# pwrliang/RayJoin

Hardware: AMD Instinct MI355X
Metric: LSI+PIP query throughput, USCounty |><| BlockGroup (higher is better)
Workload: dtype int128+f64; 1 GPU; USCounty(base, 7112768 segs) |><| BlockGroup(query, 28793160 segs, 29665680 points), -query=lsi then -query=pip, -mode=lbvh (software LBVH); kernel_schedule=k_lsi and the PIP kernels share the chip (512 + 1536 blocks), schedule_settled_before_timing=True

## Files before the change

rayjoin_amd/csrc/rj_api.hip:

```cpp
#include <hip/hip_runtime.h>
#include <rccl/rccl.h>

#include <cmath>
#include <cstdarg>
#include <cstdio>
#include <cstring>
#include <functional>
#include <new>
#include <string>
#include <thread>
#include <vector>

#include "../../include/rayjoin_amd.h"
#include "rj_crossings.h"
#include "rj_dissolve.h"
#include "rj_eliminate.h"
#include "rj_faces.h"
#include "rj_node.h"
#include "rj_kernels.h"
#include "rj_overlay_dev.h"
#include "rj_overlay_ops.h"
#include "rj_pipeline.h"
#include "rj_polygons.h"
#include "rj_ringmap.h"
// ... 1815 lines not shown
    }
  const char* why = !h->pip_walk ? "\"pip_walk\" 0: the exact kernel alone" : (walk ? "" : "instrumented (\"stats\"), no points, or more than 2^32 of them: the exact kernel alone");
  if (walk && h->pip_walk == 1 && seen != ~0ull && (seen * 10 > n * 3 || seen > 16384)) {
    walk = false;
    why = "the last two-pass query of this size left too many points to the exact kernel (> 30 %, or > 16384): first pass dropped";
  }
  const bool own = aux && walk && h->exact_own_stream;
  const int li = own ? 1 + h->exact_buf : si;
  if (walk && (h->rest_cap[si] < n || h->rest_cap[li] < n)) {
    RJ_HIP(h, hipStreamSynchronize(h->stream));
    RJ_HIP(h, join_aux(h));
    for (int k = 0; k < (h->exact_own_stream ? 3 : 2); k++) {
      if (h->rest_cap[k] >= n) continue;
      (void) hipFree(h->rest[k]); (void) hipFree(h->todo[k]); (void) hipFree(h->todo_mask[k]);
      h->rest[k] = nullptr; h->rest_cap[k] = 0; h->todo[k] = nullptr; h->todo_mask[k] = nullptr;
      if (int r = dev_alloc(h, &h->rest[k], n)) return r;
      if (int r = dev_alloc(h, &h->todo[k], n * (uint64_t) pip_walk_list_slots())) return r;
      if (int r = dev_alloc(h, &h->todo_mask[k], n / 4 + 1)) return r;
      h->rest_cap[k] = n;
      RJ_HIP(h, hipMemsetAsync(h->todo[k], 0xFF, n * (uint64_t) pip_walk_list_slots() * 4, h->stream));
      RJ_HIP(h, hipMemsetAsync(h->todo_mask[k], 0, (n / 4 + 1) * 8, h->stream));
      RJ_HIP(h, hipMemsetAsync(h->rest[k], 0, n * 4, h->stream));
    }
    RJ_HIP(h, hipStreamSynchronize(h->stream));
  }
  h->last_passes = walk ? 3 : 1;
  h->last_walk_points = 1;
  h->last_prepared = 0;
  tic(h, RJ_T_PIP_KERNEL, st);
  if (n && walk) {
    const int wflip = h->flip_walk[si];
    PipArgs w = a;
    w.work_counter = (unsigned int*) (h->d_counter + (aux ? kSchedWalkAux : kSchedWalkMain) + wflip * kSchedBlockWords);
    w.next_work_counter = (unsigned int*) (h->d_counter + (aux ? kSchedWalkAux : kSchedWalkMain) + (1 - wflip) * kSchedBlockWords);
    w.rest = h->rest[li];
    w.rest_count = h->d_counter + kRestCountWord + 2 * si + wflip;
    w.next_rest_count = h->d_counter + kRestCountWord + 2 * si + (1 - wflip);
    if (own) {
      w.rest_count = h->d_counter + kExactRestWord[h->exact_rot];
      w.next_rest_count = h->d_counter + kExactRestWord[(h->exact_rot + 1) % 3];
      h->exact_rot = (h->exact_rot + 1) % 3;
      if (h->exact_recorded[h->exact_buf]) RJ_HIP(h, hipStreamWaitEvent(st, h->ev_exact_done[h->exact_buf], 0));
      if (h->exact_last >= 0 && h->exact_recorded[h->exact_last] &&
          (h->exact_out_closest == (const void*) closest_eid_dev || (face_id_dev && h->exact_out_face == (const void*) face_id_dev)))
        RJ_HIP(h, hipStreamWaitEvent(st, h->ev_exact_done[h->exact_last], 0));
    }
    w.todo = h->todo[li]; w.todo_mask = h->todo_mask[li];
    if (!w.group_lanes) w.group_lanes = pip_walk_group_lanes(n, w.bvh.top, h->cus);
    const bool two = h->walk_points >= 2 && w.group_lanes == 64 && !h->chunk_groups && pip_walk2_blocks_per_cu(w.bvh.top) >= 6 &&
                     n >= (uint64_t) 2 * 256 * 4 * h->cus * pip_walk2_blocks_per_cu(w.bvh.top);
    tic(h, RJ_T_PIP_WALK, st);
    const bool columns = w.bvh.strips.ytab != nullptr;
    h->last_columns = columns ? 1 : 0;
    if (columns) {
      w.group_lanes = 64;
      RJ_HIP(h, launch_pip_strip(st, w, walk_blocks, h->cus));
    } else if (two) {
      if (aux && h->lsi_shared && !h->pip_share_set)
        walk_blocks = h->cus * pip_walk2_blocks_beside(w.bvh.top, walk_share_of_this_pair / h->cus < 1 ? 1 : walk_share_of_this_pair / h->cus);
      const MapState& q = h->map[query_map_id];
      if (!pts_dev && !order && !h->stats_on && q.qpts) {
        w.qpts = q.qpts + pt_begin;
        h->last_prepared = 1;
        if (pt_begin % 64 == 0) { w.qext = q.qext + pt_begin / 64; h->last_prepared = 2; }
      }
      RJ_HIP(h, launch_pip_walk2(st, w, walk_blocks, h->cus, h->stats_on));
      h->last_walk_points = 2;
    } else {
      RJ_HIP(h, launch_pip_walk(st, w, h->stats_on, walk_blocks));
    }
    if (aux && h->lsi_shared) h->last_pip_share = walk_blocks;
    h->plan.pip.first = columns ? last_strip_launch() : last_launch();
    toc(h, RJ_T_PIP_WALK, st);
    h->flip_walk[si] = 1 - wflip;
    const uint64_t left = seen != ~0ull ? seen : 8192;
    PipRestArgs r;
    r.order = h->rest[li];
    r.n_dev = w.rest_count;
    r.rest_count = h->d_rest + si;
    r.work_counter = a.work_counter;
    r.next_work_counter = a.next_work_counter;
    r.group_lanes = left < 8192 ? 1 : (left * 100 < n ? 4 : (left * 10 < n ? 8 : 16));
    r.chunk_groups = 1;
    int rest_blocks = h->cus * 4;
    if (seen != ~0ull) {
      const uint64_t want = seen / (r.group_lanes * 4 * 2) + 1;
      const uint64_t lo = (uint64_t) h->cus / 4, hi = (uint64_t) h->cus * 4;
      rest_blocks = (int) (want < lo ? lo : (want > hi ? hi : want));
    }
    r.blocks = (uint32_t) rest_blocks;
    h->walk_n[si] = n;
    if (own) {
      RJ_HIP(h, hipEventRecord(h->ev_walk_done, st));
      RJ_HIP(h, hipStreamWaitEvent(h->exact_stream, h->ev_walk_done, 0));
      RJ_HIP(h, launch_pip_exact(h->exact_stream, w, h->cus * 8, r));
      RJ_HIP(h, hipEventRecord(h->ev_exact_done[h->exact_buf], h->exact_stream));
      h->exact_recorded[h->exact_buf] = true;
      h->exact_last = h->exact_buf;
      h->exact_out_closest = closest_eid_dev; h->exact_out_face = face_id_dev;
      h->exact_buf ^= 1;
      h->exact_pending = true;
    } else {
      RJ_HIP(h, launch_pip_exact(st, w, h->cus * 8, r));
    }
    h->flip_pip[si] = 1 - pflip;
    h->plan.pip.exact_blocks = h->cus * 8; h->plan.pip.locate_blocks = rest_blocks;
    if (columns) why = "the base map has a column index (closed rings or short chains: index[].columns_why): the first pass reads the point's strip";
    else if (!two && h->walk_points >= 2) why = "one point per lane: a query set too small for full groups on every resident wave (or a debug knob set)";
  } else if (n) {
    if (aux && h->exact_pending && h->exact_last >= 0) RJ_HIP(h, hipStreamWaitEvent(st, h->ev_exact_done[h->exact_last], 0));
    RJ_HIP(h, launch_pip(st, a, h->stats_on, max_blocks));
    h->flip_pip[aux ? 1 : 0] = 1 - pflip;
    h->plan.pip.first = last_launch();
    h->plan.pip.exact_blocks = h->plan.pip.locate_blocks = 0;
  }
  {
    rj_handle_s::PlanRec::Pip& pp = h->plan.pip;
    pp.ran = n > 0; pp.epoch = h->plan.epoch; pp.n = n; pp.aux = aux; pp.caller = pts_dev != nullptr;
    pp.shared = aux && h->lsi_shared; pp.passes = h->last_passes; pp.rest_hint = seen; pp.why = why;
    pp.order = order ? (h->order_fresh ? 2 : 1) : 0;
    pp.prepared = h->last_prepared;
  }
  toc(h, RJ_T_PIP_KERNEL, own ? h->exact_stream : st);
  if (h->cur_caller >= 0 && n) {
    const rj_handle_s::CallerSet& e = h->caller[h->cur_caller];
    if (e.queries <= 2 || e.queries % 4 == 0) RJ_HIP(h, launch_group_extent_tail(st, pts, h->cur_order, n, h->d_est + h->cur_caller));
  }
  if (aux) h->aux_pending = true;
  return RJ_OK;
}

int rj_pip_query(rj_handle h, int base_map_id, int query_map_id, const int64_t* pts_dev,
                 uint64_t pt_begin, uint64_t n, uint32_t* closest_eid_dev, int32_t* face_id_dev) {
  RJ_CHECK_H(h);
  if (int r = rj_pip_query_async(h, base_map_id, query_map_id, pts_dev, pt_begin, n, closest_eid_dev, face_id_dev)) return r;
  if (h->stats_on) RJ_HIP(h, hipMemcpyAsync(h->h_pinned + 1, h->d_stats, 128, hipMemcpyDeviceToHost, h->stream));
  RJ_HIP(h, hipStreamSynchronize(h->stream));
  RJ_HIP(h, join_aux(h));
  if (h->stats_on) for (int i = 0; i < 16; i++) h->last_stats[i] = h->h_pinned[1 + i];
  return check_fault(h);
}


int rj_build_grid(rj_handle h, int map_id, int grid_size) {
  RJ_CHECK_H(h);
  if (map_id < 0 || map_id > 1 || !h->map[map_id].present) return fail(h, RJ_E_INVALID, "rj_build_grid: map %d not uploaded", map_id);
  if (grid_size < 1 || grid_size > 32768) return fail(h, RJ_E_INVALID, "rj_build_grid: grid_size must be in [1, 32768]");
  if (int r = set_device(h)) return r;
  RJ_HIP(h, join_aux(h));
  const MapState& m = h->map[map_id];
  GridState& gr = h->grid[map_id];
  free_grid(gr);
  const uint64_t ncells = (uint64_t) grid_size * grid_size;
  const double scale = (double) grid_size / (double) ((((int64_t) 1 << 46) - 1) + ((int64_t) 1 << 46)) * 0.999;
  tic(h, RJ_T_BUILD);
  uint32_t* counts = nullptr;
  uint64_t *keys = nullptr, *keys2 = nullptr;
  void* temp = nullptr;
  int rc = RJ_OK;
  hipError_t e = hipSuccess;
  do {
    if ((rc = dev_alloc(h, &counts, ncells + 1))) break;
    if ((rc = dev_alloc(h, &gr.begin, ncells + 1))) break;
    if ((e = hipMemsetAsync(counts, 0, (ncells + 1) * 4, h->stream)) != hipSuccess) break;
    if ((e = hipMemsetAsync(h->d_counter + 2, 0, 16, h->stream)) != hipSuccess) break;
    if ((e = launch_grid_count(h->stream, m.seg, m.ne, grid_size, scale, counts, h->d_counter + 2)) != hipSuccess) break;
    if ((e = hipMemcpyAsync(h->h_pinned + 26, h->d_counter + 2, 8, hipMemcpyDeviceToHost, h->stream)) != hipSuccess) break;
    if ((e = hipStreamSynchronize(h->stream)) != hipSuccess) break;
    gr.total = h->h_pinned[26];
    if (gr.total >= 0xFFFFFFFFull) {
      rc = fail(h, RJ_E_INVALID, "rj_build_grid: %llu (cell, edge) incidences do not fit 32-bit offsets: use a coarser grid",
                (unsigned long long) gr.total);
      break;
    }
    size_t scan_bytes = 0, sort_bytes = 0;
    if ((e = scan_cell_counts(h->stream, nullptr, scan_bytes, counts, gr.begin, ncells + 1)) != hipSuccess) break;
    if (gr.total && (e = sort_keys_u64(h->stream, nullptr, sort_bytes, (const uint64_t*) nullptr, (uint64_t*) nullptr, gr.total)) != hipSuccess) break;
    const size_t temp_bytes = scan_bytes > sort_bytes ? scan_bytes : sort_bytes;
    if ((e = hipMalloc(&temp, temp_bytes ? temp_bytes : 1)) != hipSuccess) break;
    size_t tb = temp_bytes;
    if ((e = scan_cell_counts(h->stream, temp, tb, counts, gr.begin, ncells + 1)) != hipSuccess) break;
    if ((rc = dev_alloc(h, &gr.eids, gr.total ? gr.total : 1))) break;
    if (gr.total) {
      if ((rc = dev_alloc(h, &keys, gr.total))) break;
      if ((rc = dev_alloc(h, &keys2, gr.total))) break;
      if ((e = launch_grid_emit(h->stream, m.seg, m.ne, grid_size, scale, keys, h->d_counter + 3)) != hipSuccess) break;
      tb = temp_bytes;
      if ((e = sort_keys_u64(h->stream, temp, tb, keys, keys2, gr.total)) != hipSuccess) break;
      if ((e = launch_grid_unpack(h->stream, keys2, gr.total, gr.eids)) != hipSuccess) break;
// ... 864 lines not shown
```

rayjoin_amd/csrc/rj_kernels.hip:

```cpp
#include "rj_kernels.h"

#include <cstring>
#include <rocprim/device/device_radix_sort.hpp>

namespace rj {

__device__ __forceinline__ uint32_t cell_code(const Seg& s) {
  const int cx0 = quant(s.x1 < s.x2 ? s.x1 : s.x2) >> kOccShift, cx1 = quant(s.x1 < s.x2 ? s.x2 : s.x1) >> kOccShift;
  const int cy0 = quant(s.y1 < s.y2 ? s.y1 : s.y2) >> kOccShift, cy1 = quant(s.y1 < s.y2 ? s.y2 : s.y1) >> kOccShift;
  const int dx = cx1 - cx0 > 1 ? 2 : cx1 - cx0, dy = cy1 - cy0 > 1 ? 2 : cy1 - cy0;
  return (uint32_t) cx0 | ((uint32_t) cy0 << 12) | ((uint32_t) dx << 24) | ((uint32_t) dy << 26);
}
__global__ __launch_bounds__(256) void k_build_segs(const int64_t* __restrict__ pts,
                                                    const uint32_t* __restrict__ edge_begin,
                                                    uint32_t nc, uint64_t ne, Seg* __restrict__ seg,
                                                    uint32_t* __restrict__ edge_chain, uint32_t* __restrict__ ccode) {
  for (uint64_t e = blockIdx.x * (uint64_t) blockDim.x + threadIdx.x; e < ne;
       e += (uint64_t) gridDim.x * blockDim.x) {
    uint32_t lo = 0, hi = nc;
    while (hi - lo > 1) {
      uint32_t mid = lo + ((hi - lo) >> 1);
      if (edge_begin[mid] <= e) lo = mid; else hi = mid;
    }
    uint64_t p = e + lo;
// ... 1124 lines not shown
}


__global__ __launch_bounds__(256) void k_xsect_keys(const XsectRec* __restrict__ rec, uint64_t n, int im,
                                                    uint64_t* __restrict__ keys, uint32_t* __restrict__ vals) {
  for (uint64_t i = blockIdx.x * (uint64_t) blockDim.x + threadIdx.x; i < n; i += (uint64_t) gridDim.x * blockDim.x) {
    const uint32_t mine = im ? rec[i].eid1 : rec[i].eid0, other = im ? rec[i].eid0 : rec[i].eid1;
    keys[i] = ((uint64_t) mine << 32) | other;
    vals[i] = (uint32_t) i;
  }
}

__global__ __launch_bounds__(256) void k_xsect_gather(const XsectRec* __restrict__ in, const uint32_t* __restrict__ order,
                                                      uint64_t n, XsectRec* __restrict__ out) {
  for (uint64_t i = blockIdx.x * (uint64_t) blockDim.x + threadIdx.x; i < n; i += (uint64_t) gridDim.x * blockDim.x)
    out[i] = in[order[i]];
}

__device__ __forceinline__ u128 xsect_dist2(const XsectRec& r, int64_t px, int64_t py) {
  const i128 dx = (i128) r.x_num - px, dy = (i128) r.y_num - py;
  return (u128) (dx * dx) + (u128) (dy * dy);
}

__global__ __launch_bounds__(256) void k_xsect_order_runs(XsectRec* __restrict__ rec, uint64_t n, int im,
                                                          const Seg* __restrict__ seg_im,
                                                          int64_t* __restrict__ midpts) {
  for (uint64_t i = blockIdx.x * (uint64_t) blockDim.x + threadIdx.x; i < n; i += (uint64_t) gridDim.x * blockDim.x) {
    const uint32_t e = im ? rec[i].eid1 : rec[i].eid0;
    if (i > 0 && (im ? rec[i - 1].eid1 : rec[i - 1].eid0) == e) continue;
    uint64_t end = i + 1;
    while (end < n && (im ? rec[end].eid1 : rec[end].eid0) == e) end++;
    const Seg s = seg_im[e];
    for (uint64_t a = i + 1; a < end; a++) {
      const XsectRec cur = rec[a];
      const u128 dc = xsect_dist2(cur, s.x1, s.y1);
      uint64_t b = a;
      while (b > i && xsect_dist2(rec[b - 1], s.x1, s.y1) > dc) {
        rec[b] = rec[b - 1];
        b--;
      }
      rec[b] = cur;
    }
    for (uint64_t a = i; a < end; a++) {
      int64_t mx = rec[a].x_num, my = rec[a].y_num;
      if (a + 1 < end) {
        mx = (int64_t) (((i128) rec[a].x_num + rec[a + 1].x_num) / 2);
        my = (int64_t) (((i128) rec[a].y_num + rec[a + 1].y_num) / 2);
      }
      midpts[2 * a] = mx;
      midpts[2 * a + 1] = my;
      rec[a].mid = -1;
    }
  }
}

__global__ __launch_bounds__(256) void k_xsect_set_mid(XsectRec* __restrict__ rec, uint64_t n, int im,
                                                       const int32_t* __restrict__ face) {
  for (uint64_t i = blockIdx.x * (uint64_t) blockDim.x + threadIdx.x; i + 1 < n; i += (uint64_t) gridDim.x * blockDim.x) {
    const uint32_t a = im ? rec[i].eid1 : rec[i].eid0, b = im ? rec[i + 1].eid1 : rec[i + 1].eid0;
    if (a == b) rec[i].mid = face[i];
  }
}

__global__ __launch_bounds__(256) void k_swap_halves(uint64_t* __restrict__ v, uint64_t n) {
  for (uint64_t i = blockIdx.x * (uint64_t) blockDim.x + threadIdx.x; i < n;
       i += (uint64_t) gridDim.x * blockDim.x) {
    uint64_t x = v[i];
    v[i] = (x << 32) | (x >> 32);
  }
}

constexpr int kPipList = 6;
#ifndef RJ_PIP_WAVES
#define RJ_PIP_WAVES 4
#endif
constexpr int kPipWaves = RJ_PIP_WAVES;
constexpr int kPipRefineAbove = 16;

struct PipWaveLds {
  uint4 stack[kPipStack];
  uint32_t cand[kPipList][64];
};

template <bool STATS>
__device__ __forceinline__ void pip_locate(const PipArgs& A, const uint32_t bid, const PipRestArgs& Q, unsigned long long* const stats) {
  __shared__ PipWaveLds lds[kPipWaves];
  const int lane = lane_id();
  const int wib = threadIdx.x >> 6;
  PipWaveLds& L = lds[wib];
  const uint32_t GL = Q.group_lanes;
  uint64_t nq = A.n;
  if (Q.n_dev) {
    const unsigned long long left = __hip_atomic_load(Q.n_dev, __ATOMIC_RELAXED, __HIP_MEMORY_SCOPE_AGENT);
    nq = left < nq ? left : nq;
    if (Q.rest_count && bid == 0 && threadIdx.x == 0) __hip_atomic_store(Q.rest_count, left, __ATOMIC_RELAXED, __HIP_MEMORY_SCOPE_SYSTEM);
  }
  const uint64_t ngroups = (nq + GL - 1) / GL;
  const DeviceBvh& T = A.bvh;
  const uint32_t* const sky = (T.sky && T.sky[kSkyBuckets] == 0u) ? T.sky : nullptr;
  const int qm = A.query_map_id;
  const int stack_cap = STATS && A.stack_cap < kPipStack ? A.stack_cap : kPipStack;
  unsigned long long st_leaf = 0, st_tests = 0, st_nodes = 0, st_box = 0;
  unsigned long long st_stale = 0, st_leaf_nocand = 0, st_leaf_lanes = 0;
  long long tk_drain = 0, tk_leaf = 0, tk_node = 0, tk_rounds = 0, tk_sched = 0, tk_head = 0, tk_tail = 0;
  const long long tk_begin = STATS ? clock64() : 0;

  const uint32_t nchunks = (uint32_t) ((ngroups + Q.chunk_groups - 1) / Q.chunk_groups);
  int part = bid & 7, tried = 0;
  __shared__ unsigned long long ranges[kPipWaves];
  if (threadIdx.x < kPipWaves) ranges[threadIdx.x] = 0;
  if (bid == 0 && threadIdx.x < 8) Q.next_work_counter[threadIdx.x * 32] = 0;
  __syncthreads();
  for (;;) {
  {
    uint32_t g32 = 0;
    const long long tks = STATS ? clock64() : 0;
    if (!next_group<kPipWaves>(ranges, wib, Q.work_counter, nchunks, Q.chunk_groups, ngroups, part, tried, lane, g32)) break;
    if (STATS) tk_sched += clock64() - tks;
    const uint64_t g = g32;
    const long long tkg = STATS ? clock64() : 0;
    const uint64_t ipos = g * GL + lane;
    const bool valid = (uint32_t) lane < GL && ipos < nq;
    const uint64_t ip = Q.order ? (valid ? Q.order[ipos] : 0) : ipos;
    int32_t qx = 0, qy = 0;
    if (valid) {
      qx = quant(A.pts[2 * ip]);
      qy = quant(A.pts[2 * ip + 1]);
    }
    const bool live = valid && ray_has_sky(sky, qx, qy);
    const int32_t qym1 = qy > 0 ? qy - 1 : 0;
    const int32_t gx0 = wave_min(live ? qx : kEmptyMin);
    const int32_t gx1 = wave_max(live ? qx : kEmptyMax);
    const int32_t gy0 = wave_min(live ? qy : kEmptyMin);
    double best_yy = __builtin_inf();
    uint32_t best_slot = 0xFFFFFFFFu;
    int32_t qbest = live ? 0x7FFFFFFF : -1;
    int32_t gbest = 0x7FFFFFFF;
    int cnt = 0;
    bool sure1 = false;
    int32_t sure_y0 = 0;

    auto evaluate = [&](bool final_round) {
      const long long tk0 = STATS ? clock64() : 0;
      if (final_round && cnt == 1 && sure1 && best_slot == 0xFFFFFFFFu) {
        best_slot = L.cand[0][lane];
        cnt = 0;
      }
      const int maxc = wave_max(cnt);
      int64_t px = 0, py = 0;
      if (cnt > 0) {
        px = A.pts[2 * ip];
        py = A.pts[2 * ip + 1];
      }
      for (int r = 0; r < maxc; r++) {
        if (r < cnt) {
          const uint32_t slot = L.cand[r][lane];
          const Seg bs = T.sseg[slot];
          double yy;
          if (pip_eval_y(bs, px, py, qm, &yy)) {
            bool better = yy < best_yy;
            if (yy == best_yy && best_slot != 0xFFFFFFFFu) {
              const Seg cur = T.sseg[best_slot];
              better = pip_better(yy, pip_slope(bs), T.seid[slot], best_yy, pip_slope(cur), T.seid[best_slot], qm);
            }
            if (better) {
              best_yy = yy; best_slot = slot;
            }
          }
        }
        if (STATS) tk_rounds++;
      }
      if (STATS) st_tests += (unsigned long long) __popcll(__ballot(cnt > 0));
      cnt = 0;
      if (final_round) {
        if (STATS) tk_drain += clock64() - tk0;
        return;
      }
      if (best_slot != 0xFFFFFFFFu && best_yy < __builtin_inf()) {
        double t = (best_yy + (double) kCoordOffset) * (1.0 / 65536.0);
        int32_t qb = t < 2147483000.0 ? (t < -1.0 ? -1 : (int32_t) t + 1) : 0x7FFFFFFF;
        qbest = qb < qbest ? qb : qbest;
      }
      gbest = wave_max(qbest);
      if (STATS) tk_drain += clock64() - tk0;
    };

    auto refine_if_many = [&](const QBox& b, uint64_t um) -> uint64_t {
      if (__popcll(um) <= kPipRefineAbove) return um;
      uint64_t keep = 0;
      while (um) {
        const int c = __builtin_ctzll(um);
        um &= um - 1;
        const int32_t cx0 = bcast(b.x0, c), cy0 = bcast(b.y0, c);
        const int32_t cx1 = bcast(b.x1, c), cy1 = bcast(b.y1, c);
        if (__ballot(ray_can_hit(qx, qym1, qbest, cx0, cy0, cx1, cy1))) keep |= 1ull << c;
      }
      return keep;
    };
    int sp = 0;
    {
// ... 49 lines not shown
        int j = want ? ub - 1 : -1;
        const int cnt_before = cnt;
        if (STATS) st_leaf_lanes += (unsigned long long) __popcll(__ballot(want));
        for (;;) {
          const int jj = j < 0 ? 0 : j;
          const int32_t pmj = __shfl(pm, jj, 64);
          const bool act = j >= 0 && pmj >= qx;
          if (!__ballot(act)) break;
          const int32_t sx0 = __shfl(bb.x0, jj, 64), sx1 = __shfl(bb.x1, jj, 64);
          const int32_t sy0 = __shfl(bb.y0, jj, 64), sy1 = __shfl(bb.y1, jj, 64);
          if (act && ray_can_hit(qx, qym1, qbest, sx0, sy0, sx1, sy1)) {
            const bool certain = sx0 < qx && qx < sx1 && sy0 > qy;
            const bool replace = certain && sure1 && cnt == 1 && sy1 < sure_y0;
            L.cand[replace ? 0 : cnt][lane] = slot0 + (uint32_t) jj;
            sure1 = replace || (cnt == 0 && certain);
            sure_y0 = sure1 ? sy0 : sure_y0;
            cnt += replace ? 0 : 1;
            if (certain && sy1 < qbest - 1) qbest = sy1 + 1;
          }
          if (STATS) st_box++;
          if (__ballot(cnt >= kPipList)) evaluate(false);
          j--;
        }
        if (STATS && !__ballot(cnt != cnt_before)) st_leaf_nocand++;
        const int32_t gbest_before = gbest;
        if (__ballot(qbest != qbest_before)) gbest = wave_max(qbest);
        if (gbest < gbest_before && sp > 1) {
          int kept = 0;
          for (int base = 0; base < sp; base += 64) {
            const int i = base + lane;
            const bool have = i < sp;
            uint4 en = make_uint4(0, 0, 0, 0);
            if (have) en = L.stack[i];
            const bool alive = have && (int32_t) en.y <= gbest;
            const uint64_t am = __ballot(alive);
            wave_lds_fence();
            if (alive) L.stack[kept + rank_below(am)] = en;
            kept += __popcll(am);
          }
          if (STATS) st_stale += (unsigned long long) (sp - kept);
          sp = kept;
          wave_lds_fence();
        }
        if (STATS) tk_leaf += (clock64() - tk0) - (tk_drain - tkd0);
      }
    }
    const long long tkt = STATS ? clock64() : 0;
    evaluate(true);
    if (valid) {
      const bool hit = best_slot != 0xFFFFFFFFu;
      __builtin_nontemporal_store(hit ? T.seid[best_slot] : 0xFFFFFFFFu, A.closest + ip);
      if (A.face) __builtin_nontemporal_store(hit ? T.sface[best_slot] : 0, A.face + ip);
    }
    if (STATS) tk_tail += clock64() - tkt;
  }
  }
  if (STATS && lane == 0 && stats) {
    const long long tk_total = clock64() - tk_begin;
    atomicAdd(&stats[0], st_leaf);
    atomicAdd(&stats[1], st_tests);
    atomicAdd(&stats[2], st_nodes);
    atomicAdd(&stats[3], st_box);
    atomicAdd(&stats[4], (unsigned long long) tk_total);
    atomicAdd(&stats[5], (unsigned long long) tk_node);
    atomicAdd(&stats[6], (unsigned long long) tk_leaf);
    atomicAdd(&stats[7], (unsigned long long) tk_drain);
    atomicAdd(&stats[8], (unsigned long long) tk_rounds);
    atomicMax(&stats[9], (unsigned long long) tk_total);
    atomicAdd(&stats[10], (unsigned long long) tk_sched);
    atomicAdd(&stats[11], (unsigned long long) tk_head);
    atomicAdd(&stats[12], (unsigned long long) tk_tail);
    atomicAdd(&stats[13], st_stale);
    atomicAdd(&stats[14], st_leaf_nocand);
    atomicAdd(&stats[15], st_leaf_lanes);
  }
}

template <bool STATS>
__global__ __launch_bounds__(64 * kPipWaves, 6) void k_pip(PipArgs A) {
  PipRestArgs Q;
  Q.order = A.order; Q.n_dev = A.n_dev; Q.rest_count = A.rest_count;
  Q.work_counter = A.work_counter; Q.next_work_counter = A.next_work_counter;
  Q.group_lanes = A.group_lanes; Q.chunk_groups = A.chunk_groups; Q.blocks = 0;
  pip_locate<STATS>(A, blockIdx.x, Q, A.stats);
}


constexpr int kWalkStack = 124;
__host__ __device__ __forceinline__ int walk_stack_entries(int top) {
  const int worst = 64 + 63 * (top > 1 ? top - 1 : 0) + 3;
  return worst < kWalkStack ? worst : kWalkStack;
}
__host__ __device__ __forceinline__ size_t walk_wave_lds(int top) { return (size_t) 16 * walk_stack_entries(top) + (size_t) kWalkList * 256; }

template <bool STATS>
__global__ __launch_bounds__(256, 8) void k_pip_walk(PipArgs A) {
  extern __shared__ uint4 walk_smem[];
  const int lane = lane_id();
  const int wib = threadIdx.x >> 6;
  const DeviceBvh& T = A.bvh;
  const uint32_t* const sky = (T.sky && T.sky[kSkyBuckets] == 0u) ? T.sky : nullptr;
  const int stack_entries = walk_stack_entries(T.top);
  const int stack_cap = A.walk_stack > 0 && A.walk_stack < stack_entries ? A.walk_stack : stack_entries;
  uint4* const stack = walk_smem + (size_t) wib * (walk_wave_lds(T.top) / 16);
  uint32_t* const cand = reinterpret_cast<uint32_t*>(stack + stack_entries);
  const uint32_t stack_lds = (uint32_t) (uintptr_t) stack;
  const uint32_t GL = A.group_lanes;
  const uint64_t ngroups = (A.n + GL - 1) / GL;
  const uint32_t nchunks = (uint32_t) ((ngroups + A.chunk_groups - 1) / A.chunk_groups);
  int part = blockIdx.x & 7, tried = 0;
  unsigned long long st_leaf = 0, st_nodes = 0, st_box = 0, st_stale = 0, st_rest = 0, st_leaf_lanes = 0;
  long long tk_leaf = 0, tk_node = 0, tk_sched = 0, tk_head = 0, tk_tail = 0;
  const long long tk_begin = STATS ? clock64() : 0;
  __shared__ unsigned long long ranges[4];
  if (threadIdx.x < 4) ranges[threadIdx.x] = 0;
  if (blockIdx.x == 0 && threadIdx.x < 8) A.next_work_counter[threadIdx.x * 32] = 0;
  if (blockIdx.x == 0 && threadIdx.x == 8) *A.next_rest_count = 0;
  __syncthreads();
  for (;;) {
    uint32_t g32 = 0;
    const long long tks = STATS ? clock64() : 0;
    if (!next_group<4>(ranges, wib, A.work_counter, nchunks, A.chunk_groups, ngroups, part, tried, lane, g32)) break;
    if (STATS) tk_sched += clock64() - tks;
    const long long tkg = STATS ? clock64() : 0;
    const uint64_t ipos = (uint64_t) g32 * GL + lane;
    const bool valid = (uint32_t) lane < GL && ipos < A.n;
    const uint64_t ipc = valid ? ipos : A.n - 1;
    const uint32_t ip = A.order ? A.order[ipc] : (uint32_t) ipc;
    typedef long long ll2_t __attribute__((ext_vector_type(2)));
    const ll2_t pt_raw = __builtin_nontemporal_load(reinterpret_cast<const ll2_t*>(A.pts) + ip);
    const QBox root_box = T.lvl[T.top][lane];
    const uint64_t root_higher = sibling_order(T, T.top)[lane];
    const int32_t qx = valid ? quant(pt_raw.x) : 0, qy = valid ? quant(pt_raw.y) : 0;
    const bool live = valid && ray_has_sky(sky, qx, qy);
    const int32_t qym1 = qy > 0 ? qy - 1 : 0;
    int32_t gx0 = live ? qx : kEmptyMin, gx1 = live ? qx : kEmptyMax, gy0 = live ? qy : kEmptyMin;
    wave_min_max_min(gx0, gx1, gy0);
    int32_t qbest = live ? 0x7FFFFFFF : -1;
    int32_t gbest = 0x7FFFFFFF;
    const uint32_t cand_base = (uint32_t) lane;
    uint32_t cand_at = cand_base;
    int32_t sure_y0 = INT32_MIN;

    auto refine_if_many = [&](const QBox& b, uint64_t um) -> uint64_t {
      if (__popcll(um) <= kPipRefineAbove) return um;
      uint64_t keep = 0;
      while (um) {
        const int c = __builtin_ctzll(um);
        um &= um - 1;
        const int32_t cx0 = bcast(b.x0, c), cy0 = bcast(b.y0, c);
        const int32_t cx1 = bcast(b.x1, c), cy1 = bcast(b.y1, c);
        if (__ballot(ray_can_hit(qx, qym1, qbest, cx0, cy0, cx1, cy1))) keep |= 1ull << c;
      }
      return keep;
    };
    int sp = 0, sp_max = 0;
    bool ovf = false;
    {
      const QBox b = root_box;
      const uint64_t higher = root_higher;
      uint64_t m = refine_if_many(b, __ballot(b.x0 <= gx1 && gx0 <= b.x1 && b.y1 >= gy0 - 1));
      if (__popcll(m) > stack_cap) { m = 0; ovf = true; }
      if ((m >> lane) & 1)
        stack[__popcll(m & higher)] = make_uint4(((uint32_t) T.top << 28) | (uint32_t) lane, (uint32_t) b.y0, (uint32_t) b.x0, (uint32_t) b.x1);
      sp = __popcll(m);
      sp_max = sp;
      wave_lds_fence();
// ... 458 lines not shown
      const int32_t f = A.face ? T.sface[slot] : 0;
      out_e[p] = hit ? e : 0xFFFFFFFFu;
      out_f[p] = hit ? f : 0;
    }
#pragma unroll
    for (int p = 0; p < P; p++) {
      const uint32_t fill = (cand_at[p] - cand_base[p]) >> 6;
      const bool listed = valid[p] && !donev[p] && !ovf && fill <= (uint32_t) kWalkList;
      const bool rest = valid[p] && !donev[p] && !listed;
      const uint64_t lm = __ballot(listed);
      const uint64_t g64 = (uint64_t) g32 * P + p;
      if (listed) {
        const uint64_t rec = g64 * 64 + rank_below(lm);
#pragma unroll
        for (int k = 0; k < kWalkList; k++) A.todo[rec * kWalkList + k] = (uint32_t) k < fill ? cand[cand_base[p] + 64 * k] : 0xFFFFFFFFu;
      }
      if (lane == 0 && g64 * 64 < A.n) A.todo_mask[g64] = lm;
      const uint64_t rm = __ballot(rest);
      if (rm) {
        unsigned long long base = 0;
        if (lane == 0) base = atomicAdd(A.rest_count, (unsigned long long) __popcll(rm));
        base = ((unsigned long long) __builtin_amdgcn_readfirstlane((uint32_t) (base >> 32)) << 32) | __builtin_amdgcn_readfirstlane((uint32_t) base);
        if (rest) A.rest[base + rank_below(rm)] = ipv[p];
      }
      if (STATS) st_rest += (unsigned long long) __popcll(rm);
    }
#pragma unroll
    for (int p = 0; p < P; p++) {
      if (donev[p]) {
        __builtin_nontemporal_store(out_e[p], A.closest + ipv[p]);
        if (A.face) __builtin_nontemporal_store(out_f[p], A.face + ipv[p]);
      }
    }
    wave_lds_fence();
    if (STATS && cyc) { asm volatile("s_waitcnt vmcnt(0)" ::: "memory"); RJ_CK(ck_tail, ck); }
  }
#undef RJ_CK
  if (STATS && A.stats && cyc) {
    if (lane == 0) {
      const long long total = clock64() - ck_begin;
      atomicAdd(&A.stats[0], (unsigned long long) total);
      atomicAdd(&A.stats[1], (unsigned long long) ck_sched);
      atomicAdd(&A.stats[2], (unsigned long long) ck_load);
      atomicAdd(&A.stats[3], (unsigned long long) ck_head);
      atomicAdd(&A.stats[4], st_groups);
      atomicAdd(&A.stats[5], (unsigned long long) ck_pop);
      atomicAdd(&A.stats[6], (unsigned long long) ck_node_wait);
      atomicAdd(&A.stats[7], (unsigned long long) ck_node);
      atomicAdd(&A.stats[8], (unsigned long long) ck_leaf_wait);
      atomicAdd(&A.stats[9], (unsigned long long) ck_leaf);
      atomicAdd(&A.stats[10], (unsigned long long) ck_bound);
      atomicAdd(&A.stats[11], (unsigned long long) ck_tail);
      atomicAdd(&A.stats[12], 1ull);
    }
    return;
  }
  if (STATS && A.stats) {
    const unsigned long long hits = st_hits;
    if (hits) atomicAdd(&A.stats[6], hits);
    if (lane == 0) {
      atomicAdd(&A.stats[0], st_leaf);
      atomicAdd(&A.stats[1], st_rest);
      atomicAdd(&A.stats[2], st_nodes);
      atomicAdd(&A.stats[3], st_steps);
      atomicAdd(&A.stats[4], st_groups);
      atomicAdd(&A.stats[5], st_setvisits);
      atomicAdd(&A.stats[7], st_sweeps);
      atomicAdd(&A.stats[8], st_swept);
      atomicAdd(&A.stats[10], st_pops);
      atomicAdd(&A.stats[11], st_pushed);
      atomicAdd(&A.stats[13], st_stale);
      atomicAdd(&A.stats[15], st_want);
    }
  }
}


__global__ __launch_bounds__(256, 8) __attribute__((amdgpu_num_sgpr(96))) __attribute__((amdgpu_num_vgpr(28))) void k_pip_walk2(PipArgs A) { pip_walk_many<false, 2>(A); }
__global__ __launch_bounds__(256, 4) __attribute__((amdgpu_num_sgpr(96))) void k_pip_walk2_stats(PipArgs A) { pip_walk_many<true, 2>(A); }
__global__ __launch_bounds__(256, 8) __attribute__((amdgpu_num_sgpr(96))) __attribute__((amdgpu_num_vgpr(28))) void k_pip_walk2_prepared(PipArgs A) { pip_walk_many<false, 2, true>(A); }


#ifndef RJ_EXACT_WAVES
#define RJ_EXACT_WAVES 5
#endif
static_assert(kPipWaves == 4, "k_pip_exact's first blocks run pip_locate: same block size");
__global__ __launch_bounds__(256, RJ_EXACT_WAVES) void k_pip_exact(PipArgs A, PipRestArgs R) {
  if (blockIdx.x < R.blocks) {
    pip_locate<false>(A, blockIdx.x, R, nullptr);
    return;
  }
  __shared__ uint32_t queue[4][128];
  __shared__ uint32_t qrec[4][128];
  const DeviceBvh& T = A.bvh;
  const int lane = lane_id();
  const int wib = threadIdx.x >> 6;
  const uint32_t gl_shift = 31 - __builtin_clz(A.group_lanes);
  const uint64_t wave = ((blockIdx.x - R.blocks) * (uint64_t) blockDim.x + threadIdx.x) >> 6;
  const uint64_t nwaves = ((uint64_t) (gridDim.x - R.blocks) * blockDim.x) >> 6;
  auto evaluate = [&](uint32_t i, uint32_t rec) {
    const uint64_t ip = A.order ? A.order[i] : i;
    uint32_t slot[kWalkList];
#pragma unroll
    for (int r = 0; r < kWalkList; r++) slot[r] = A.todo[(uint64_t) rec * kWalkList + r];
    typedef long long ll2_t __attribute__((ext_vector_type(2)));
    const ll2_t pxy = reinterpret_cast<const ll2_t*>(A.pts)[ip];
    const int64_t px = pxy.x, py = pxy.y;
    double best_yy = __builtin_inf();
    uint32_t best_slot = 0xFFFFFFFFu;
    Seg best_seg = {0, 0, 0, 0};
    int64_t best_lo = INT64_MAX, best_hi = INT64_MAX;
    bool best_exact = false;
    Seg cur = {0, 0, 0, 0}, nxt = {0, 0, 0, 0};
    if (slot[0] != 0xFFFFFFFFu) cur = T.sseg[slot[0]];
    if (slot[1] != 0xFFFFFFFFu) nxt = T.sseg[slot[1]];
#pragma unroll
    for (int r = 0; r < kWalkList; r++) {
      if (slot[r] == 0xFFFFFFFFu) break;
      const Seg e = cur;
      cur = nxt;
      if (r + 2 < kWalkList && slot[r + 2] != 0xFFFFFFFFu) nxt = T.sseg[slot[r + 2]];
      const int64_t x_min = e.x1 < e.x2 ? e.x1 : e.x2, x_max = e.x1 < e.x2 ? e.x2 : e.x1;
      if (px < x_min || px > x_max || px == (A.query_map_id == 0 ? x_min : x_max)) continue;
      const int64_t ylo = e.y1 < e.y2 ? e.y1 : e.y2, yhi = e.y1 < e.y2 ? e.y2 : e.y1;
      if (yhi <= py - 1) continue;
      if (ylo >= py + 1 && ylo > best_hi) continue;
      if (ylo >= py + 1 && yhi < best_lo) {
        best_slot = slot[r]; best_seg = e; best_lo = ylo; best_hi = yhi; best_exact = false;
        continue;
      }
      if (best_slot != 0xFFFFFFFFu && !best_exact) {
        double byy;
        (void) pip_eval_y(best_seg, px, py, A.query_map_id, &byy);
        best_yy = byy; best_exact = true;
      }
      double yy;
      if (pip_eval_y(e, px, py, A.query_map_id, &yy)) {
        bool better = yy < best_yy;
        if (yy == best_yy && best_slot != 0xFFFFFFFFu)
          better = pip_better(yy, pip_slope(e), T.seid[slot[r]], best_yy, pip_slope(best_seg), T.seid[best_slot], A.query_map_id);
        if (better) {
          best_yy = yy; best_slot = slot[r]; best_seg = e; best_lo = ylo; best_hi = yhi; best_exact = true;
        }
      }
    }
    const bool hit = best_slot != 0xFFFFFFFFu;
    A.closest[ip] = hit ? T.seid[best_slot] : 0xFFFFFFFFu;
    if (A.face) A.face[ip] = hit ? T.sface[best_slot] : 0;
  };
  int nq = 0;
  const uint64_t ngroups = (A.n + A.group_lanes - 1) >> gl_shift;
  for (uint64_t g0 = wave * 16; g0 < ngroups; g0 += nwaves * 16) {
    unsigned long long mine = 0;
    if (lane < 16 && g0 + lane < ngroups) mine = A.todo_mask[g0 + lane];
    uint64_t any = __ballot(mine != 0);
    while (any) {
      const int k = __builtin_ctzll(any);
      any &= any - 1;
      const uint64_t m = ((uint64_t) (uint32_t) __builtin_amdgcn_readlane((int) (mine >> 32), k) << 32) |
                         (uint32_t) __builtin_amdgcn_readlane((int) mine, k);
      if ((m >> lane) & 1) {
        const uint32_t r = rank_below(m);
        queue[wib][nq + r] = (uint32_t) (((g0 + k) << gl_shift) + lane);
        qrec[wib][nq + r] = (uint32_t) ((g0 + k) << gl_shift) + r;
      }
      nq += __popcll(m);
      wave_lds_fence();
      if (nq >= 64) {
        evaluate(queue[wib][nq - 64 + lane], qrec[wib][nq - 64 + lane]);
        nq -= 64;
        wave_lds_fence();
      }
    }
  }
  if (lane < nq) evaluate(queue[wib][lane], qrec[wib][lane]);
}

__global__ void k_noop() {}
hipError_t warm_query_kernels(hipStream_t st) {
  hipLaunchKernelGGL(k_noop, dim3(1), dim3(1), 0, st);
  return hipGetLastError();
}

static thread_local LaunchNote g_note = {"", 0, 0};
LaunchNote last_launch() { return g_note; }
static inline void note(const char* kernel, int grid, int per_lane) { g_note.kernel = kernel; g_note.grid = grid; g_note.per_lane = per_lane; }

static inline int grid_for(uint64_t work_items, int per_block, int max_blocks) {
  uint64_t b = (work_items + per_block - 1) / per_block;
  if (b < 1) b = 1;
  if (b > (uint64_t) max_blocks) b = max_blocks;
  return (int) b;
}

hipError_t launch_build_segs(hipStream_t st, const int64_t* pts, const uint32_t* edge_begin,
                             uint32_t nc, uint64_t ne, Seg* seg, uint32_t* edge_chain, uint32_t* ccode) {
  if (ne == 0) return hipSuccess;
  hipLaunchKernelGGL(k_build_segs, dim3(grid_for(ne, 256, 8192)), dim3(256), 0, st, pts, edge_begin,
                     nc, ne, seg, edge_chain, ccode);
  return hipGetLastError();
}

hipError_t launch_prepare_points(hipStream_t st, const int64_t* pts, uint64_t np, int2* qpts, int4* qext) {
  if (np == 0) return hipSuccess;
  hipLaunchKernelGGL(k_prepare_points, dim3(grid_for(np, 256, 8192)), dim3(256), 0, st, pts, np, qpts, qext);
  return hipGetLastError();
}

hipError_t launch_morton(hipStream_t st, const Seg* seg, uint64_t ne, MortonKey* keys, uint32_t* vals) {
  if (ne == 0) return hipSuccess;
  hipLaunchKernelGGL(k_morton, dim3(grid_for(ne, 256, 8192)), dim3(256), 0, st, seg, ne, keys, vals);
  return hipGetLastError();
}

hipError_t sort_pairs_u64_u32(hipStream_t st, void* temp, size_t& temp_bytes, const uint64_t* kin,
                              uint64_t* kout, const uint32_t* vin, uint32_t* vout, uint64_t n, unsigned begin_bit,
                              unsigned end_bit) {
  return rocprim::radix_sort_pairs(temp, temp_bytes, kin, kout, vin, vout, (size_t) n, begin_bit, end_bit, st);
}

hipError_t sort_morton_pairs(hipStream_t st, void* temp, size_t& temp_bytes, const MortonKey* kin, MortonKey* kout,
                             const uint32_t* vin, uint32_t* vout, uint64_t n) {
  return rocprim::radix_sort_pairs(temp, temp_bytes, kin, kout, vin, vout, (size_t) n, 0, 64 - kMortonDropBits, st);
}

hipError_t sort_keys_u64(hipStream_t st, void* temp, size_t& temp_bytes, const uint64_t* kin,
                         uint64_t* kout, uint64_t n) {
  return rocprim::radix_sort_keys(temp, temp_bytes, kin, kout, (size_t) n, 0, 64, st);
}

hipError_t launch_xsect_keys(hipStream_t st, const XsectRec* rec, uint64_t n, int im, uint64_t* keys, uint32_t* vals) {
  if (n) hipLaunchKernelGGL(k_xsect_keys, dim3(grid_for(n, 256, 4096)), dim3(256), 0, st, rec, n, im, keys, vals);
  return hipGetLastError();
}
hipError_t launch_xsect_gather(hipStream_t st, const XsectRec* in, const uint32_t* order, uint64_t n, XsectRec* out) {
  if (n) hipLaunchKernelGGL(k_xsect_gather, dim3(grid_for(n, 256, 4096)), dim3(256), 0, st, in, order, n, out);
  return hipGetLastError();
}
hipError_t launch_xsect_order_runs(hipStream_t st, XsectRec* rec, uint64_t n, int im, const Seg* seg_im, int64_t* midpts) {
  if (n) hipLaunchKernelGGL(k_xsect_order_runs, dim3(grid_for(n, 256, 4096)), dim3(256), 0, st, rec, n, im, seg_im, midpts);
  return hipGetLastError();
}
hipError_t launch_xsect_set_mid(hipStream_t st, XsectRec* rec, uint64_t n, int im, const int32_t* face) {
// ... 270 lines not shown
```

Baseline: 39960 M query segments/s.

## Run PIP locate blocks as single waves and trim exact-kernel registers for occupancy

The locate part of k_pip_exact now runs with one active wave per block using a shared LDS union, and the grid gets four times more locate blocks with a lower divisor. The exact evaluator drops its prefetch-ahead segment and its cached y bounds (recomputed from best_seg), and reads the todo mask from LDS instead of via readlane. Launch bounds rise from five to six waves. The aim is to cut VGPR pressure and LDS footprint so more waves are resident alongside the LSI kernel. The cost is less memory-latency hiding from the shorter prefetch, and 3 of 4 waves exiting right away in each locate block.

Measured after the change: 39850 M query segments/s. Within noise of the previous version (-0.3%).

```diff
diff --git a/rayjoin_amd/csrc/rj_api.hip b/rayjoin_amd/csrc/rj_api.hip
--- a/rayjoin_amd/csrc/rj_api.hip
+++ b/rayjoin_amd/csrc/rj_api.hip
@@ -1921,18 +1921,19 @@
     r.next_work_counter = a.next_work_counter;
     r.group_lanes = left < 8192 ? 1 : (left * 100 < n ? 4 : (left * 10 < n ? 8 : 16));
     r.chunk_groups = 1;
-    int rest_blocks = h->cus * 4;
+    int rest_blocks = h->cus * 16;
     if (seen != ~0ull) {
-      const uint64_t want = seen / (r.group_lanes * 4 * 2) + 1;
-      const uint64_t lo = (uint64_t) h->cus / 4, hi = (uint64_t) h->cus * 4;
+      const uint64_t want = seen / (r.group_lanes * 2) + 1;
+      const uint64_t lo = (uint64_t) h->cus, hi = (uint64_t) h->cus * 16;
       rest_blocks = (int) (want < lo ? lo : (want > hi ? hi : want));
     }
     r.blocks = (uint32_t) rest_blocks;
+    const int exact_blocks = h->cus * 8;
     h->walk_n[si] = n;
     if (own) {
       RJ_HIP(h, hipEventRecord(h->ev_walk_done, st));
       RJ_HIP(h, hipStreamWaitEvent(h->exact_stream, h->ev_walk_done, 0));
-      RJ_HIP(h, launch_pip_exact(h->exact_stream, w, h->cus * 8, r));
+      RJ_HIP(h, launch_pip_exact(h->exact_stream, w, exact_blocks, r));
       RJ_HIP(h, hipEventRecord(h->ev_exact_done[h->exact_buf], h->exact_stream));
       h->exact_recorded[h->exact_buf] = true;
       h->exact_last = h->exact_buf;
@@ -1940,10 +1941,10 @@
       h->exact_buf ^= 1;
       h->exact_pending = true;
     } else {
-      RJ_HIP(h, launch_pip_exact(st, w, h->cus * 8, r));
+      RJ_HIP(h, launch_pip_exact(st, w, exact_blocks, r));
     }
     h->flip_pip[si] = 1 - pflip;
-    h->plan.pip.exact_blocks = h->cus * 8; h->plan.pip.locate_blocks = rest_blocks;
+    h->plan.pip.exact_blocks = exact_blocks; h->plan.pip.locate_blocks = rest_blocks;
     if (columns) why = "the base map has a column index (closed rings or short chains: index[].columns_why): the first pass reads the point's strip";
     else if (!two && h->walk_points >= 2) why = "one point per lane: a query set too small for full groups on every resident wave (or a debug knob set)";
   } else if (n) {
diff --git a/rayjoin_amd/csrc/rj_kernels.hip b/rayjoin_amd/csrc/rj_kernels.hip
--- a/rayjoin_amd/csrc/rj_kernels.hip
+++ b/rayjoin_amd/csrc/rj_kernels.hip
@@ -1230,11 +1230,11 @@
   uint32_t cand[kPipList][64];
 };
 
-template <bool STATS>
-__device__ __forceinline__ void pip_locate(const PipArgs& A, const uint32_t bid, const PipRestArgs& Q, unsigned long long* const stats) {
-  __shared__ PipWaveLds lds[kPipWaves];
+template <bool STATS, int NW>
+__device__ __forceinline__ void pip_locate(const PipArgs& A, const uint32_t bid, const PipRestArgs& Q, unsigned long long* const stats,
+                                           PipWaveLds* const lds, unsigned long long* const ranges) {
   const int lane = lane_id();
-  const int wib = threadIdx.x >> 6;
+  const int wib = NW > 1 ? threadIdx.x >> 6 : 0;
   PipWaveLds& L = lds[wib];
   const uint32_t GL = Q.group_lanes;
   uint64_t nq = A.n;
@@ -1255,15 +1255,14 @@
 
   const uint32_t nchunks = (uint32_t) ((ngroups + Q.chunk_groups - 1) / Q.chunk_groups);
   int part = bid & 7, tried = 0;
-  __shared__ unsigned long long ranges[kPipWaves];
-  if (threadIdx.x < kPipWaves) ranges[threadIdx.x] = 0;
+  if (threadIdx.x < NW) ranges[threadIdx.x] = 0;
   if (bid == 0 && threadIdx.x < 8) Q.next_work_counter[threadIdx.x * 32] = 0;
-  __syncthreads();
+  if (NW > 1) __syncthreads(); else wave_lds_fence();
   for (;;) {
   {
     uint32_t g32 = 0;
     const long long tks = STATS ? clock64() : 0;
-    if (!next_group<kPipWaves>(ranges, wib, Q.work_counter, nchunks, Q.chunk_groups, ngroups, part, tried, lane, g32)) break;
+    if (!next_group<NW>(ranges, wib, Q.work_counter, nchunks, Q.chunk_groups, ngroups, part, tried, lane, g32)) break;
     if (STATS) tk_sched += clock64() - tks;
     const uint64_t g = g32;
     const long long tkg = STATS ? clock64() : 0;
@@ -1479,7 +1478,9 @@
   Q.order = A.order; Q.n_dev = A.n_dev; Q.rest_count = A.rest_count;
   Q.work_counter = A.work_counter; Q.next_work_counter = A.next_work_counter;
   Q.group_lanes = A.group_lanes; Q.chunk_groups = A.chunk_groups; Q.blocks = 0;
-  pip_locate<STATS>(A, blockIdx.x, Q, A.stats);
+  __shared__ PipWaveLds lds[kPipWaves];
+  __shared__ unsigned long long ranges[kPipWaves];
+  pip_locate<STATS, kPipWaves>(A, blockIdx.x, Q, A.stats, lds, ranges);
 }
 
 
@@ -2104,16 +2105,30 @@
 
 
 #ifndef RJ_EXACT_WAVES
-#define RJ_EXACT_WAVES 5
+#define RJ_EXACT_WAVES 6
 #endif
-static_assert(kPipWaves == 4, "k_pip_exact's first blocks run pip_locate: same block size");
+struct ExactLocateLds {
+  PipWaveLds wave;
+  unsigned long long ranges[1];
+};
+struct ExactQueueLds {
+  uint32_t queue[4][128];
+  uint32_t qrec[4][128];
+  unsigned long long mask[4][16];
+};
+constexpr size_t kExactLds = sizeof(ExactLocateLds) > sizeof(ExactQueueLds) ? sizeof(ExactLocateLds) : sizeof(ExactQueueLds);
+static_assert(kExactLds <= 8192, "k_pip_exact: LDS must not decide its occupancy");
 __global__ __launch_bounds__(256, RJ_EXACT_WAVES) void k_pip_exact(PipArgs A, PipRestArgs R) {
+  __shared__ __attribute__((aligned(16))) unsigned char lds_raw[kExactLds];
   if (blockIdx.x < R.blocks) {
-    pip_locate<false>(A, blockIdx.x, R, nullptr);
+    if (threadIdx.x >= 64) return;
+    ExactLocateLds& LL = *reinterpret_cast<ExactLocateLds*>(lds_raw);
+    pip_locate<false, 1>(A, blockIdx.x, R, nullptr, &LL.wave, LL.ranges);
     return;
   }
-  __shared__ uint32_t queue[4][128];
-  __shared__ uint32_t qrec[4][128];
+  ExactQueueLds& QL = *reinterpret_cast<ExactQueueLds*>(lds_raw);
+  uint32_t (&queue)[4][128] = QL.queue;
+  uint32_t (&qrec)[4][128] = QL.qrec;
   const DeviceBvh& T = A.bvh;
   const int lane = lane_id();
   const int wib = threadIdx.x >> 6;
@@ -2131,24 +2146,24 @@
     double best_yy = __builtin_inf();
     uint32_t best_slot = 0xFFFFFFFFu;
     Seg best_seg = {0, 0, 0, 0};
-    int64_t best_lo = INT64_MAX, best_hi = INT64_MAX;
     bool best_exact = false;
-    Seg cur = {0, 0, 0, 0}, nxt = {0, 0, 0, 0};
+    Seg cur = {0, 0, 0, 0};
     if (slot[0] != 0xFFFFFFFFu) cur = T.sseg[slot[0]];
-    if (slot[1] != 0xFFFFFFFFu) nxt = T.sseg[slot[1]];
 #pragma unroll
     for (int r = 0; r < kWalkList; r++) {
       if (slot[r] == 0xFFFFFFFFu) break;
       const Seg e = cur;
-      cur = nxt;
-      if (r + 2 < kWalkList && slot[r + 2] != 0xFFFFFFFFu) nxt = T.sseg[slot[r + 2]];
+      if (r + 1 < kWalkList && slot[r + 1] != 0xFFFFFFFFu) cur = T.sseg[slot[r + 1]];
       const int64_t x_min = e.x1 < e.x2 ? e.x1 : e.x2, x_max = e.x1 < e.x2 ? e.x2 : e.x1;
       if (px < x_min || px > x_max || px == (A.query_map_id == 0 ? x_min : x_max)) continue;
       const int64_t ylo = e.y1 < e.y2 ? e.y1 : e.y2, yhi = e.y1 < e.y2 ? e.y2 : e.y1;
       if (yhi <= py - 1) continue;
+      const bool have = best_slot != 0xFFFFFFFFu;
+      const int64_t best_lo = have ? (best_seg.y1 < best_seg.y2 ? best_seg.y1 : best_seg.y2) : INT64_MAX;
+      const int64_t best_hi = have ? (best_seg.y1 < best_seg.y2 ? best_seg.y2 : best_seg.y1) : INT64_MAX;
       if (ylo >= py + 1 && ylo > best_hi) continue;
       if (ylo >= py + 1 && yhi < best_lo) {
-        best_slot = slot[r]; best_seg = e; best_lo = ylo; best_hi = yhi; best_exact = false;
+        best_slot = slot[r]; best_seg = e; best_exact = false;
         continue;
       }
       if (best_slot != 0xFFFFFFFFu && !best_exact) {
@@ -2162,7 +2177,7 @@
         if (yy == best_yy && best_slot != 0xFFFFFFFFu)
           better = pip_better(yy, pip_slope(e), T.seid[slot[r]], best_yy, pip_slope(best_seg), T.seid[best_slot], A.query_map_id);
         if (better) {
-          best_yy = yy; best_slot = slot[r]; best_seg = e; best_lo = ylo; best_hi = yhi; best_exact = true;
+          best_yy = yy; best_slot = slot[r]; best_seg = e; best_exact = true;
         }
       }
     }
@@ -2173,14 +2188,20 @@
   int nq = 0;
   const uint64_t ngroups = (A.n + A.group_lanes - 1) >> gl_shift;
   for (uint64_t g0 = wave * 16; g0 < ngroups; g0 += nwaves * 16) {
-    unsigned long long mine = 0;
-    if (lane < 16 && g0 + lane < ngroups) mine = A.todo_mask[g0 + lane];
-    uint64_t any = __ballot(mine != 0);
+    uint64_t any;
+    {
+      unsigned long long mine = 0;
+      if (lane < 16 && g0 + lane < ngroups) mine = A.todo_mask[g0 + lane];
+      if (lane < 16) QL.mask[wib][lane] = mine;
+      any = __ballot(mine != 0);
+      wave_lds_fence();
+    }
     while (any) {
       const int k = __builtin_ctzll(any);
       any &= any - 1;
-      const uint64_t m = ((uint64_t) (uint32_t) __builtin_amdgcn_readlane((int) (mine >> 32), k) << 32) |
-                         (uint32_t) __builtin_amdgcn_readlane((int) mine, k);
+      const unsigned long long mk = QL.mask[wib][k];
+      const uint64_t m = ((uint64_t) (uint32_t) __builtin_amdgcn_readfirstlane((int) (mk >> 32)) << 32) |
+                         (uint32_t) __builtin_amdgcn_readfirstlane((int) mk);
       if ((m >> lane) & 1) {
         const uint32_t r = rank_below(m);
         queue[wib][nq + r] = (uint32_t) (((g0 + k) << gl_shift) + lane);
```
